# batra-mlp-lab/visdial

Measured on AMD Instinct MI355X. Metric: QA-rounds/sec training mn-att-ques-im-hist+disc (batch 20x10x100), higher is better.
Workload: dtype f32 operands and results; the option recurrence multiplies the EXACT 3-way bf16 split of both operands (9 bf16 MFMA products per fp32 product, f32 accumulate: fp32-grade, errors at the f32 MFMA's own level) -- its two step kernels and its weight-gradient contraction; f32 MFMA (v_mfma_f32_32x32x2_f32

## Files before the change

### visdial_amd/csrc/common.h

```cpp
#pragma once
#include <hip/hip_runtime.h>
#include <stdint.h>
#include <stdio.h>
#include <string.h>

#define VD_OK 0
#define VD_ERR_ARG -1
#define VD_ERR_HIP -2
#define VD_ERR_STATE -3
#define VD_FLAG_BF16 1
#define VD_FLAG_SPLIT9 2
#define VD_FLAG_SPLIT6 4
#define VD_FLAG_SPLIT3 8
#define VD_FLAG_SPLIT (VD_FLAG_SPLIT9 | VD_FLAG_SPLIT6 | VD_FLAG_SPLIT3)
#define VD_FLAG_LIVE_PREFIX 16
#define VD_FLAG_STATE_ONLY 32
#define VD_FLAG_TREE 64
#define VD_LIVE_PREFIX_ROWS 128

void vd_set_error(const char* fmt, ...);

#define VD_CHECK_ARG(cond, ...)                                   \
  do {                                                            \
    if (!(cond)) {                                                \
// ... 41 lines not shown
  int n;
  long quads_per_row;
};
int vd_zero_inactive_multi(const VdZeroSet& z, const int32_t* nact_dev, int T, int N, hipStream_t stream);

typedef unsigned short vd_bf16_bits;
int vd_lstm_forward_c16(const vd_bf16_bits* table16, int64_t tab_ld, const int32_t* tok_gather, const float* Wh, vd_bf16_bits* gates16,
                        vd_bf16_bits* h16, float* h_last, float* c, int T, int N, int H, hipStream_t stream);
int vd_lstm_backward_c16(const float* Wh, vd_bf16_bits* gates16, const float* c, const float* dh_last, float* dc_work, int T, int N, int H,
                         hipStream_t stream);
int vd_f32_to_bf16(const float* src, vd_bf16_bits* dst, int64_t n, hipStream_t stream);
int vd_gemm_tn_acc_bf16(const vd_bf16_bits* A16, const vd_bf16_bits* B16, float* C, int64_t ldc, int M, int N, int K, hipStream_t stream);
int vd_segment_rowsum_acc_bf16(const vd_bf16_bits* X16, int64_t ldx, const int32_t* tok, const int32_t* perm, int64_t n, int ncol,
                               float* out, int64_t ldo, hipStream_t stream);

int vd_bf16_shadow_get(int slot, const float* base, size_t floats, vd_bf16_bits** out);
const vd_bf16_bits* vd_bf16_shadow_find(const float* p, size_t floats);
void vd_bf16_shadow_invalidate(const float* p, size_t floats);

typedef float f32x16 __attribute__((ext_vector_type(16)));

__device__ __forceinline__ float vd_rcp(float x) { return __builtin_amdgcn_rcpf(x); }
__device__ __forceinline__ float vd_sigmoid(float x) { return vd_rcp(1.0f + __expf(-x)); }
__device__ __forceinline__ float vd_tanh(float x) {
  const float e = __expf(-2.0f * fabsf(x));
  const float t = (1.0f - e) * vd_rcp(1.0f + e);
  return copysignf(t, x);
}

typedef unsigned vd_u32x4 __attribute__((ext_vector_type(4)));
// ... 59 lines not shown
```

### visdial_amd/csrc/elementwise.hip

```cpp
#include <stdlib.h>

#include "common.h"

__device__ __forceinline__ uint32_t mix32(uint64_t x) {
  x ^= x >> 33;
  x *= 0xff51afd7ed558ccdULL;
  x ^= x >> 33;
  x *= 0xc4ceb9fe1a85ec53ULL;
  x ^= x >> 33;
  return (uint32_t)x;
}

__global__ void dropout_mask_kernel(uint8_t* __restrict__ mask, long n, uint64_t seed, float p) {
  const long i4 = ((long)blockIdx.x * blockDim.x + threadIdx.x) * 4;
  if (i4 >= n) return;
  const uint32_t thr = (uint32_t)(p * 16777216.0f);
  uint8_t m[4];
#pragma unroll
  for (int k = 0; k < 4; ++k) {
    const uint32_t h = mix32(seed * 0x9E3779B97F4A7C15ULL + (uint64_t)(i4 + k));
    m[k] = ((h >> 8) >= thr) ? 1 : 0;
  }
  if (i4 + 3 < n) {
    *reinterpret_cast<uint32_t*>(mask + i4) = m[0] | (m[1] << 8) | (m[2] << 16) | ((uint32_t)m[3] << 24);
// ... 109 lines not shown
  unsigned long long todo = __ballot(active);
  const int lane = threadIdx.x & 63;
  while (todo) {
    const int leader = __ffsll((long long)todo) - 1;
    const int ltok = __shfl(tok, leader, 64);
    const unsigned long long same = __ballot(active && tok == ltok) & todo;
    int basev = 0;
    if (lane == leader) basev = atomicAdd(base + ltok, __popcll(same));
    basev = __shfl(basev, leader, 64);
    if ((same >> lane) & 1ULL) result = basev + __popcll(same & ((1ULL << lane) - 1ULL));
    todo &= ~same;
  }
  return result;
}

__global__ void tok_count_kernel(const int* __restrict__ tok, long n, int* __restrict__ count) {
  const long i = (long)blockIdx.x * blockDim.x + threadIdx.x;
  const bool active = i < n;
  wave_agg_atomic_inc(count, active ? tok[i] : 0, active);
}

__global__ void tok_scan_kernel(const int* __restrict__ count, int V, int* __restrict__ offset,
                                int* __restrict__ cursor) {
  __shared__ int part[1024];
  const int tid = threadIdx.x, nt = blockDim.x;
  const int per = (V + nt - 1) / nt;
  const int b = tid * per, e = min(V, b + per);
  int s = 0;
  for (int i = b; i < e; ++i) s += count[i];
  part[tid] = s;
  __syncthreads();
  if (tid == 0) {
    int run = 0;
    for (int i = 0; i < nt; ++i) {
      const int t = part[i];
      part[i] = run;
      run += t;
    }
    offset[V] = run;
  }
  __syncthreads();
  int run = part[tid];
  for (int i = b; i < e; ++i) {
    offset[i] = run;
    cursor[i] = run;
    run += count[i];
  }
}

__global__ void tok_fill_kernel(const int* __restrict__ tok, long n, int* __restrict__ cursor,
                                int* __restrict__ perm) {
  const long i = (long)blockIdx.x * blockDim.x + threadIdx.x;
  const bool active = i < n;
  const int p = wave_agg_atomic_inc(cursor, active ? tok[i] : 0, active);
  if (active) perm[p] = (int)i;
}

template <int CHUNK, bool X16 = false>
__global__ void __launch_bounds__(256)
segment_rowsum_kernel(const float* __restrict__ X, long ldx, const int* __restrict__ tok,
                      const int* __restrict__ perm, long n, int ncol, float* __restrict__ out, long ldo) {
  __shared__ int srow[CHUNK], stok[CHUNK];
  const long p0 = (long)blockIdx.x * CHUNK;
  if (p0 >= n) return;
  const int cnt = (int)min((long)CHUNK, n - p0);
  if ((int)threadIdx.x < cnt) {
    const int r = perm[p0 + threadIdx.x];
    srow[threadIdx.x] = r;
    stok[threadIdx.x] = tok[r];
// ... 194 lines not shown
                    float scale, void* stream);
}
int vd_zero_inactive_multi(const VdZeroSet& z, const int32_t* nact_dev, int T, int N, hipStream_t stream) {
  VD_CHECK_ARG(z.n >= 1 && z.n <= 6 && nact_dev && T >= 0 && N >= 0, "vd_zero_inactive_multi: bad args");
  if (T == 0 || N == 0) return VD_OK;
  VdZeroSet zz = z;
  zz.quads_per_row = 0;
  for (int i = 0; i < z.n; ++i) {
    VD_CHECK_ARG(z.buf[i] && z.ncols[i] % 4 == 0, "vd_zero_inactive_multi: buffer %d", i);
    zz.quads_per_row += z.ncols[i] >> 2;
  }
  hipLaunchKernelGGL(zero_inactive_multi_kernel, dim3(128, T), dim3(256), 0, stream, zz, nact_dev, N);
  VD_LAUNCH_CHECK();
  return VD_OK;
}
extern "C" {
int vd_embed_gather(const float* emb, const int32_t* tok, const uint8_t* mask, float* out, int64_t rows, int E,
                    float scale, void* stream) {
  VD_CHECK_ARG(emb && tok && out && rows >= 0 && E > 0 && E % 4 == 0, "vd_embed_gather: bad args (E=%d)", E);
  if (rows == 0) return VD_OK;
  hipLaunchKernelGGL(embed_gather_kernel, grid1d(rows * (E / 4), 256), dim3(256), 0, (hipStream_t)stream, emb,
                     tok, mask, out, (long)rows, E, scale);
  VD_LAUNCH_CHECK();
  return VD_OK;
}

int vd_embed_scatter_acc(float* demb, const int32_t* tok, const uint8_t* mask, const float* dx, int64_t rows,
                         int E, float scale, void* stream) {
  VD_CHECK_ARG(demb && tok && dx && rows >= 0 && E > 0, "vd_embed_scatter_acc: bad args");
  if (rows == 0) return VD_OK;
  hipLaunchKernelGGL(embed_scatter_kernel, grid1d(rows * E, 256), dim3(256), 0, (hipStream_t)stream, demb, tok,
                     mask, dx, (long)rows, E, scale);
  VD_LAUNCH_CHECK();
  return VD_OK;
}

int vd_token_sort(const int32_t* tok, int64_t n, int V, int32_t* offset, int32_t* work, int32_t* perm,
                  void* stream) {
  VD_CHECK_ARG(tok && offset && work && perm && n >= 0 && V > 0, "vd_token_sort: bad args");
  hipStream_t s = (hipStream_t)stream;
  int* count = work;
  int* cursor = work + V;
  VD_HIP(hipMemsetAsync(count, 0, sizeof(int) * V, s));
  if (n > 0) {
    hipLaunchKernelGGL(tok_count_kernel, grid1d(n, 256), dim3(256), 0, s, tok, (long)n, count);
    VD_LAUNCH_CHECK();
  }
  hipLaunchKernelGGL(tok_scan_kernel, dim3(1), dim3(1024), 0, s, count, V, offset, cursor);
  VD_LAUNCH_CHECK();
  if (n > 0) {
    hipLaunchKernelGGL(tok_fill_kernel, grid1d(n, 256), dim3(256), 0, s, tok, (long)n, cursor, perm);
    VD_LAUNCH_CHECK();
  }
  return VD_OK;
}

int vd_segment_rowsum_acc(const float* X, int64_t ldx, const int32_t* tok, const int32_t* perm, int64_t n,
                          int ncol, float* out, int64_t ldo, void* stream) {
  VD_CHECK_ARG(X && tok && perm && out && n >= 0 && ncol > 0 && ncol % 4 == 0 && ldx % 4 == 0 && ldo % 4 == 0,
               "vd_segment_rowsum_acc: bad args");
  if (n == 0) return VD_OK;
  hipLaunchKernelGGL(segment_rowsum_kernel<256>, grid1d(n, 256), dim3(256), 0, (hipStream_t)stream, X, (long)ldx, tok, perm, (long)n, ncol,
                     out, (long)ldo);
  VD_LAUNCH_CHECK();
  return VD_OK;
}

int vd_clamp_adam(float* w, float* g, float* m, float* v, int64_t n, float gscale, float clip, float beta1,
                  float beta2, float eps, float step, void* stream) {
  VD_CHECK_ARG(w && g && m && v && n >= 0, "vd_clamp_adam: bad args");
  VD_CHECK_ARG((((uintptr_t)w | (uintptr_t)g | (uintptr_t)m | (uintptr_t)v) & 15) == 0,
               "vd_clamp_adam: buffers must be 16-byte aligned");
  if (n == 0) return VD_OK;
  hipLaunchKernelGGL(clamp_adam_kernel, grid1d((n + 3) / 4, 256), dim3(256), 0, (hipStream_t)stream, w, g, m, v,
                     (long)n, gscale, clip, beta1, beta2, eps, step);
  VD_LAUNCH_CHECK();
  return VD_OK;
}

}

int vd_segment_rowsum_acc_bf16(const vd_bf16_bits* X16, int64_t ldx, const int32_t* tok, const int32_t* perm, int64_t n, int ncol,
                               float* out, int64_t ldo, hipStream_t stream) {
  VD_CHECK_ARG(X16 && tok && perm && out && n >= 0 && ncol % 4 == 0 && ldx % 4 == 0, "vd_segment_rowsum_acc_bf16: bad args");
  if (n == 0) return VD_OK;
  hipLaunchKernelGGL((segment_rowsum_kernel<256, true>), grid1d(n, 256), dim3(256), 0, stream, reinterpret_cast<const float*>(X16), (long)ldx,
                     tok, perm, (long)n, ncol, out, (long)ldo);
  VD_LAUNCH_CHECK();
  return VD_OK;
}
```

### visdial_amd/csrc/lstm.hip

```cpp
#include "gemm_core.h"
#include "split_core.h"

extern "C" int vd_gemm_tn_acc(const float* A, int64_t lda, const float* B, int64_t ldb, float* C, int64_t ldc, int M,
                              int N, int K, int flags, void* stream);

template <int SEQ, bool C16 = false>
struct EpiLstmFwdT {
  const float* xproj;
  long xld;
  const int* tok_gather;
  const int* tok_mask;
  const float* c_prev;
  float* gates;
  float* c_out;
  float* h_out;
  int H;
  vd_bf16_bits* h16 = nullptr;
  __device__ __forceinline__ void sequential(const f32x16 (&acc)[4], int row0, int vcol0, int lane, int M, float* scr) const {
    const int j = (vcol0 >> 7) * 32 + (lane & 7) * 4;
    float4 ai[4], af[4], ao[4], ag[4];
    tile_to_rows(acc[0], scr, lane, ai);
    tile_to_rows(acc[1], scr, lane, af);
    tile_to_rows(acc[2], scr, lane, ao);
    tile_to_rows(acc[3], scr, lane, ag);
// ... 396 lines not shown
      L.g16[3] = __builtin_amdgcn_raw_buffer_load_b64(R.g, og4 >> 1, 3 * (uH4 >> 1), 0);
    } else {
    L.g[0] = vd_buf_ld4(R.g, og4, 0);
    L.g[1] = vd_buf_ld4(R.g, og4, uH4);
    L.g[2] = vd_buf_ld4(R.g, og4, 2 * uH4);
    L.g[3] = vd_buf_ld4(R.g, og4, 3 * uH4);
    }
    L.ct = vd_buf_ld4(R.ct, o4, 0);
    const float4 z = make_float4(0.f, 0.f, 0.f, 0.f);
    L.cp = c_prev ? vd_buf_ld4(R.cp, o4, 0) : z;
    L.dcv = dc_first ? z : vd_buf_ld4(R.dc, o4, 0);
    L.dhx = (dh_a || dh_b) ? vd_buf_ld4(R.dh1, o4, 0) : z;
  }
  __device__ __forceinline__ void operator()(const f32x16 (&acc)[NT], int row0, int col0, int lane, int M,
                                             int N, float* scr) const {
    const int rl = lane >> 3, cl = (lane & 7) * 4;
    const bool two_dh = TWO && dh_a && dh_b;
    const Rsrc R{vd_rsrc(gates), vd_rsrc(c_t), vd_rsrc(c_prev), vd_rsrc(dc), vd_rsrc(dh_a ? dh_a : dh_b), vd_rsrc(dh_b), vd_rsrc(da16)};
    const unsigned uH4 = (unsigned)H * 4u;
#pragma unroll
    for (int jt = 0; jt < NT; ++jt) {
      float4 d4[4];
      tile_to_rows(acc[jt], scr, lane, d4);
      if (jt == 0) VD_T(3);
      const int j = col0 + jt * 32 + cl;
      const int jc = j < N ? j : N - 4;
#pragma unroll
      for (int pp = 0; pp < 4; pp += BATCH) {
        Slot L[BATCH];
        unsigned o4[BATCH], og4[BATCH];
#pragma unroll
        for (int q = 0; q < BATCH; ++q) {
          const int row = row0 + (pp + q) * 8 + rl;
          o4[q] = (unsigned)(row < M ? row : M - 1) * uH4 + (unsigned)jc * 4u;
          og4[q] = 4u * o4[q] - 12u * (unsigned)jc;
          load_slot_buf(L[q], R, o4[q], og4[q], uH4);
        }
        __builtin_amdgcn_sched_barrier(0);
#pragma unroll
        for (int q = 0; q < BATCH; ++q) {
          Slot& C = L[q];
// ... 38 lines not shown
              vd_buf_st4_bf16(R.g, og4[q] >> 1, 3 * (uH4 >> 1), ag);
            } else {
            vd_buf_st4(R.g, og4[q], 0, ai);
            vd_buf_st4(R.g, og4[q], uH4, af);
            vd_buf_st4(R.g, og4[q], 2 * uH4, ao);
            vd_buf_st4(R.g, og4[q], 3 * uH4, ag);
            }
            vd_buf_st4(R.dc, o4[q], 0, dn);
            if (!C16 && da16) {
              vd_buf_st4_bf16(R.g16, og4[q] >> 1, 0, ai);
              vd_buf_st4_bf16(R.g16, og4[q] >> 1, uH4 >> 1, af);
              vd_buf_st4_bf16(R.g16, og4[q] >> 1, uH4, ao);
              vd_buf_st4_bf16(R.g16, og4[q] >> 1, 3 * (uH4 >> 1), ag);
            }
          }
        }
      }
    }
  }
};

using CfgF9 = GemmCfg<4, 1, 4, 16, 0, 4, 41984>;
using CfgB1 = GemmCfg<4, 1, 4, 32, 0, 3>;
using CfgB11 = GemmCfg<4, 1, 2, 16, 0, 4, 41984>;
using CfgFbf16 = GemmCfg<4, 1, 4, 32, 0, 3, 0, 1>;
using CfgBbf16 = GemmCfg<4, 1, 2, 32, 0, 3, 0, 1>;
#ifndef VD_C16_LDS
#define VD_C16_LDS 41984
#endif
using CfgF9bf16 = GemmCfg<4, 1, 4, 16, 0, 4, VD_C16_LDS, 1>;
using CfgB11bf16 = GemmCfg<4, 1, 2, 16, 0, 4, VD_C16_LDS, 1>;
using CfgFwdSmallA = GemmCfg<1, 4, 4, 8, 0, 3>;
using CfgFwdSmallC = GemmCfg<1, 4, 4, 8, 0, 4>;
using CfgBwdSmallD = GemmCfg<1, 4, 1, 32, 2, 4>;
using CfgTickFwdBf16 = GemmCfg<1, 4, 4, 16, 0, 3, 0, 1>;
using CfgTickBwdBf16 = GemmCfg<1, 4, 1, 32, 0, 4, 0, 1>;

__global__ void __launch_bounds__(256) wh_gate_transpose_kernel(const float* __restrict__ Wh,
                                                                float* __restrict__ WhT, int H, int plain = 0) {
// ... 36 lines not shown
  SrcKGate4 b{Wh, 4L * H, H};
  if (N >= VD_THROUGHPUT_ROWS) return launch_gemm<CfgF9>(N, 4 * H, K, 1, a, b, epi, s);
  return launch_gemm<CfgFwdSmallA>(N, 4 * H, K, 1, a, b, epi, s);
}

static int lstm_step_fwd_tree(const float* h_prev, const float* Wh, int N, int H, const EpiLstmFwdTree& epi, hipStream_t s) {
  SrcRowTree a{h_prev, H, epi.tok_mask, epi.parent};
  SrcKGate4 b{Wh, 4L * H, H};
  if (N >= VD_THROUGHPUT_ROWS) return launch_gemm<CfgF9>(N, 4 * H, H, 1, a, b, epi, s);
  return launch_gemm<CfgFwdSmallA>(N, 4 * H, H, 1, a, b, epi, s);
}

static int lstm_step_bwd(const float* da_next, const float* Wh, int N, int H, int K, const float* dh_a,
                         const float* dh_b, float* gates, const float* c_t, const float* c_prev, float* dc,
                         int dc_first, hipStream_t s, int split = 0, const vd_bf16_bits* W3 = nullptr, vd_bf16_bits* da16 = nullptr,
                         const vd_bf16_bits* da16_next = nullptr, const vd_bf16_bits* Wh16 = nullptr) {
  SrcRow a{da_next, 4L * H};
  SrcRow b{Wh, 4L * H};
  if (split && K > 0 && !(dh_a && dh_b)) {
    EpiLstmBwd<4, 2, false> e{dh_a, dh_b, gates, c_t, c_prev, dc, dc_first, H};
    if (split == 9) return launch_gemm_split<9>(N, H, K, da_next, 4L * H, W3, 4L * H, 4L * H * H, e, s);
    if (split == 6) return launch_gemm_split<6>(N, H, K, da_next, 4L * H, W3, 4L * H, 4L * H * H, e, s);
    return launch_gemm_split<3>(N, H, K, da_next, 4L * H, W3, 4L * H, 4L * H * H, e, s);
  }
  if (da16 && K > 0) {
    EpiLstmBwd<2> e{dh_a, dh_b, gates, c_t, c_prev, dc, dc_first, H, da16};
    if (da16_next && Wh16 && K % 32 == 0)
      return launch_gemm_glds<CfgB11bf16, false>(N, H, K / 2, 1, reinterpret_cast<const float*>(da16_next), 2L * H,
                                                 reinterpret_cast<const float*>(Wh16), 2L * H, e, s);
    return launch_gemm<CfgBbf16>(N, H, K, 1, a, b, e, s);
  }
  if (da16) {
    EpiLstmBwd<2> e{dh_a, dh_b, gates, c_t, c_prev, dc, dc_first, H, da16};
// ... 297 lines not shown
      rc = launch_gemm_split<6>(N, 4 * H, H, hp, (long)H, W3, (long)H, 4L * H * H, e, s);
    else if (split == 3)
      rc = launch_gemm_split<3>(N, 4 * H, H, hp, (long)H, W3, (long)H, 4L * H * H, e, s);
    else if (glds)
      rc = launch_gemm_glds<CfgF9, false>(N, 4 * H, H, 1, hp, (long)H, WhT, (long)H, e, s);
    else
      rc = lstm_step_fwd(hp, Wh, N, H, H, e, s);
    if (rc) return rc;
  }
  return VD_OK;
}

int vd_lstm_backward(const float* Wh, float* gates, const float* c, const float* c0, const float* dh_seq,
                     const float* dh_last, const float* dc_last, float* dc_work, float* dh0, const float* h_seq,
                     float* dWh_acc, int T, int N, int H, int flags, void* stream) {
  VD_CHECK_ARG(T >= 1 && N >= 0 && H > 0 && H % 32 == 0, "vd_lstm_backward: bad dims T=%d N=%d H=%d", T, N, H);
  VD_CHECK_ARG(Wh && gates && c && dc_work, "vd_lstm_backward: null pointer");
  VD_CHECK_ARG((h_seq == nullptr) == (dWh_acc == nullptr), "vd_lstm_backward: h_seq and dWh_acc go together");
  VD_CHECK_ARG((long)N * 4 * H * 4 < (1L << 32), "vd_lstm_backward: N=%d rows x 4H=%d exceed 4 GB per step: split the batch", N, 4 * H);
  hipStream_t s = (hipStream_t)stream;
  const long NH = (long)N * H;
  if (dc_last && dc_last != dc_work) VD_HIP(hipMemcpyAsync(dc_work, dc_last, NH * sizeof(float), hipMemcpyDeviceToDevice, s));
  const bool bf16 = (flags & VD_FLAG_BF16) && vd_lstm_bf16_fits(N, H);
  const int split = !bf16 && T > 1 && vd_lstm_glds_bwd_fits(N, H) ? vd_split_nprod(flags) : 0;
  vd_bf16_bits* da16 = nullptr;
  vd_bf16_bits* Wh16 = nullptr;
  if (bf16) {
    if (int rc0 = vd_bf16_shadow_get(1, gates, (size_t)T * 4 * NH, &da16)) return rc0;
    if (T > 1) {
      VdStreamScratch wscr;
      if (int rc0 = vd_stream_scratch(s, (size_t)4 * H * H * 6, 0, &wscr)) return rc0;
// ... 4 lines not shown
    vd_bf16_shadow_invalidate(gates, (size_t)T * 4 * NH);
  }
  const vd_bf16_bits* W3 = nullptr;
  if (split) {
    VdStreamScratch wscr;
    if (int rc0 = vd_stream_scratch(s, (size_t)4 * H * H * 10, 0, &wscr)) return rc0;
    vd_bf16_bits* w3 = reinterpret_cast<vd_bf16_bits*>(wscr.wht + (size_t)4 * H * H);
    if (int rc0 = weights_to_bf16x3(Wh, w3, 4L * H * H, s)) return rc0;
    W3 = w3;
  }
  for (int t = T - 1; t >= 0; --t) {
    const bool last = (t == T - 1);
    const float* da_next = last ? nullptr : gates + (long)(t + 1) * 4 * NH;
    const int rc = lstm_step_bwd(da_next, Wh, N, H, last ? 0 : 4 * H, dh_seq ? dh_seq + t * NH : nullptr, (last && dh_last) ? dh_last : nullptr,
                                 gates + (long)t * 4 * NH, c + t * NH, t ? c + (t - 1) * NH : c0, dc_work, (last && !dc_last) ? 1 : 0, s, split,
                                 W3, da16 ? da16 + (long)t * 4 * NH : nullptr, (da16 && !last) ? da16 + (long)(t + 1) * 4 * NH : nullptr, Wh16);
    if (rc) return rc;
  }
  int rc = VD_OK;
  if (dWh_acc && T > 1) {
    rc = vd_gemm_tn_acc(h_seq, H, gates + 4 * NH, 4L * H, dWh_acc, 4L * H, H, 4 * H, (T - 1) * N, flags & (VD_FLAG_BF16 | VD_FLAG_SPLIT9), s);
    if (rc) return rc;
  }
  if (dh0) {
    SrcRow a{gates, 4L * H};
    SrcRow b{Wh, 4L * H};
    EpiStore<4> e{dh0, H, nullptr, VD_ACT_NONE, 0};
    rc = launch_gemm<CfgB1>(N, H, 4 * H, 1, a, b, e, s);
    if (rc) return rc;
  }
  return VD_OK;
}

}

template <class Cfg>
static int lstm2_forward_ticks(const vd_lstm2_fwd_t* st, int nstacks, int H, int Tmax, hipStream_t stream) {
  for (int tau = 0; tau < Tmax + 2; ++tau) {
    GroupArgs<TickFwdProb, 3 * VD_MAX_STACKS> g;
    g.nprob = 0;
    for (int s = 0; s < nstacks; ++s) {
      const vd_lstm2_fwd_t& S = st[s];
      const long NH = (long)S.N * H;
      for (int layer = 1; layer <= 2; ++layer) {
        const int t = layer == 1 ? tau : tau - 2;
        if (t < 0 || t >= S.T) continue;
        float* gates = layer == 1 ? S.gates1 : S.gates2;
        float* h = layer == 1 ? S.h1 : S.h2;
        float* c = layer == 1 ? S.c1 : S.c2;
// ... 133 lines not shown
```

### visdial_amd/csrc/paths.h

```cpp
#pragma once
#include "common.h"

static inline int vd_precision_flags(int lstmBf16) {
  switch (lstmBf16) {
    case 0: return 0;
    case 1: return VD_FLAG_BF16;
    case 3: return VD_FLAG_SPLIT3;
    case 6: return VD_FLAG_SPLIT6;
    case 9: return VD_FLAG_SPLIT9;
    default: return -1;
  }
}
static inline int vd_split_nprod(int flags) {
  return (flags & VD_FLAG_SPLIT9) ? 9 : (flags & VD_FLAG_SPLIT6) ? 6 : (flags & VD_FLAG_SPLIT3) ? 3 : 0;
}

constexpr long VD_THROUGHPUT_ROWS = 2048;
constexpr int VD_LSTM_FWD_TILE_BIG = 128, VD_LSTM_FWD_TILE_SMALL = 32;
static inline int vd_lstm_fwd_row_tile(long N) { return N >= VD_THROUGHPUT_ROWS ? VD_LSTM_FWD_TILE_BIG : VD_LSTM_FWD_TILE_SMALL; }
static inline bool vd_lstm_glds_fwd_fits(long N, int H) { return N >= VD_THROUGHPUT_ROWS && H % 32 == 0 && N * H * 4 < (1L << 32); }
static inline bool vd_lstm_glds_bwd_fits(long N, int H) { return N >= VD_THROUGHPUT_ROWS && H % 32 == 0 && N * 4 * H * 4 < (1L << 32); }
static inline bool vd_lstm_bf16_fits(long N, int H) { return N >= VD_THROUGHPUT_ROWS && H % 32 == 0; }
static inline bool vd_lstm_c16_fits(long N, int H) { return N >= VD_THROUGHPUT_ROWS && H % 128 == 0; }

static inline bool vd_tn_kmajor_fits(long M, long N, long K) { return M % 128 == 0 && N % 128 == 0 && K >= 1024; }
constexpr int VD_SPLIT_TN_BM = 256, VD_SPLIT_TN_BN = 128;
static inline bool vd_tn_split_tiles(long M, long N) { return M % VD_SPLIT_TN_BM == 0 && N % VD_SPLIT_TN_BN == 0; }

static inline bool vd_img_split_ok(long rows, int H, int Kc) {
  return rows >= 128 && H % 16 == 0 && Kc % 16 == 0 && rows * (H > Kc ? H : Kc) * 4 < (1L << 32);
}

static inline bool vd_lhood_fused_fits(long rows, long ldh, long V, long ldw, int H) {
  return H >= 64 && H % 16 == 0 && V >= 128 && ldh % 4 == 0 && ldw % 4 == 0 && rows * ldh * 4 < (1L << 32) && V * ldw * 4 < (1L << 32);
}
static inline bool vd_lhood_prefix_fits(int T, long rows) { return T >= 1 && T < 256 && rows >= 1; }
// ... 1 lines not shown
```

### visdial_amd/csrc/rt_core.h

```cpp
#pragma once
#include <math.h>
#include <stdarg.h>
#include <stdlib.h>
#include <string.h>

#include <algorithm>
#include <map>
#include <memory>
#include <numeric>
#include <random>
#include <string>
#include <vector>

#include "../../include/visdial_hip.h"
#include "common.h"
#include "paths.h"

int vd_lstm2_forward_p(const vd_lstm2_fwd_t* st, int nstacks, int H, int flags, hipStream_t stream);
int vd_lstm2_backward_p(const vd_lstm2_bwd_t* st, int nstacks, int H, int flags, hipStream_t stream);

int vd_img_drop_gather(const float* pre, const uint8_t* mask1, float* xdrop, int N, int R, int S2, int H, float scale, hipStream_t stream);
int vd_img_common_forward_p(const float* pre, const uint8_t* mask1, const float* xdrop, const float* Wc, const float* bc, const float* qc,
                            const uint8_t* mask2, float* iqc, int N, int R, int S2, int H, int Kc, float scale, int flags, hipStream_t stream);
int vd_img_tr_backward_p(const float* dz, const float* Wc, const float* p, const float* datt, const uint8_t* mask1, float* dpre, int N, int R,
// ... 53 lines not shown
  int32_t *enode = nullptr, *etgt = nullptr;
};

struct BatchSlot {
  int B = 0;
  bool tree_ok = false;
  std::vector<TreeChunk> tree;
  SeqTok q, h, opt, ain, aout, oin, oout;
  float* img = nullptr;
  int32_t* gt = nullptr;
  std::vector<int32_t> gt_host;
  bool has_gt = false;
  int32_t* opt_uid = nullptr;
  int opt_total = 0;
  int32_t *opt_sort_off = nullptr, *opt_sort_perm = nullptr;
  bool cached = false;
  uint64_t cache_stamp = 0;
  std::vector<int32_t> miss_keys, opt_host;
  hipEvent_t ready = nullptr;
  hipEvent_t done = nullptr;
  bool used = false;
  bool uploaded = false;
  std::map<std::string, DevBuf> bufs, pinned;
};

struct RowIndex {
  int T = 0;
  std::vector<int32_t> keys;
  std::vector<int32_t> table;
  int32_t size() const { return T ? (int32_t)(keys.size() / (size_t)T) : 0; }
// ... 476 lines not shown
```

### visdial_amd/csrc/rt_decoders.h

```cpp
#pragma once
#include "rt_encoders.h"

namespace vdrt {

int option_cache_resolve(vd_model* m, BatchSlot& sl, const int32_t* options, long NO, int To, hipStream_t s);

struct Decoder {
  virtual ~Decoder() {}
  virtual void declare(vd_model* m) = 0;
  virtual int forward_backward(vd_model* m, BatchSlot& b, bool only_forward) = 0;
  virtual int retrieve(vd_model* m, BatchSlot& b) = 0;
  virtual int retrieve_lhood(vd_model*, BatchSlot&) {
    vd_set_error("vd_model_retrieve_lhood: the live-row log-likelihood head scores candidates of decoder 'gen'; this model's decoder is 'disc'");
    return VD_ERR_ARG;
  }
  virtual int gen_begin(vd_model*, const int32_t*, int) { return no_gen(); }
  virtual int gen_step(vd_model*, const int32_t*, float*) { return no_gen(); }
  virtual int gen_select(vd_model*, const int32_t*, int) { return no_gen(); }
  virtual int gen_beam_search(vd_model*, int, int, int, int, int32_t*, double*) { return no_gen(); }
  virtual int gen_sample(vd_model*, int, int, int, double, const double*, int32_t*, double*) { return no_gen(); }
  static int no_gen() {
    vd_set_error("sampling / beam search only for the generative decoder (model.lua:436-438)");
    return VD_ERR_STATE;
  }
// ... 88 lines not shown
    VD_TRY(vd_score_ce(optH, enc_out, b.gt, scores, loss_rows, dedup ? d_optH_full : d_optH, d_enc, N, O, (int)H, 1.0f / N, s));
    if (dedup && !only_forward) {
      VD_TRY(vd_memset(d_optH, 0, (long)NO * H * 4, s));
      VD_TRY(vd_embed_scatter_acc(d_optH, b.opt_uid, nullptr, d_optH_full, NOfull, (int)H, 1.f, s));
    }
    VD_TRY(stage_loss(m, loss_rows, N, false, s));
    m->scores = scores;
    m->prof_valid = !only_forward;
    if (only_forward) return VD_OK;
    VD_TRY(fork_stream(m, s, se));
    float *dc, *dtab;
    int32_t* perm = b.opt_sort_perm;
    VD_TRY(ws_get(m, "opt.dc", (size_t)NO * H, &dc));
    VD_TRY(ws_get(m, "opt.dtable", (size_t)(V + 1) * 4 * H, &dtab));
    VD_CHECK_ARG(perm, "decoder 'disc': the batch slot carries no option-token sort");
    VD_TRY(fork_stream(m, s, st));
    VD_TRY(vd_memset(dtab, 0, (V + 1) * 4 * H * 4, st));
    VD_HIP(hipEventRecord(m->ev_prof[2], s));
    m->wg_active = m->streams && m->s_wg && (flags & VD_FLAG_BF16) != 0;
    m->wg_used = false;
    auto enc_bwd = [&]() -> int {
      VdRange r("encoder backward");
      VD_TRY(m->enc->backward(m, se, b, d_enc));
      VD_PROBE_REC(1, se);
      if (m->wg_used) VD_PROBE_REC(2, m->s_wg);
      if (m->wg_used) {
        VD_TRY(fork_stream(m, se, m->s_wg));
        VD_HIP(hipEventRecord(m->ev_enc_grads, m->s_wg));
      } else {
        VD_HIP(hipEventRecord(m->ev_enc_grads, se));
      }
      m->enc_grads_recorded = true;
      return VD_OK;
    };
    {
      VdRange r("disc: option LSTM backward");
      if (c16) VD_TRY(vd_lstm_backward_c16(Wopt + E * 4 * H, gates16, c, d_optH, dc, To, NO, (int)H, s));
      else VD_TRY(vd_lstm_backward(Wopt + E * 4 * H, gates, c, nullptr, nullptr, d_optH, nullptr, dc, nullptr, nullptr, nullptr, To, NO, (int)H, flags, s));
    }
    VD_HIP(hipEventRecord(m->ev_prof[3], s));
    VD_TRY(enc_bwd());
    VdRange rwg("disc: table gradient + dWh");
    VD_TRY(fork_stream(m, s, st));
    if (c16) VD_TRY(vd_segment_rowsum_acc_bf16(gates16, 4 * H, b.opt.tok, perm, (long)To * NO, (int)(4 * H), dtab, 4 * H, st));
    else VD_TRY(vd_segment_rowsum_acc(gates, 4 * H, b.opt.tok, perm, (long)To * NO, (int)(4 * H), dtab, 4 * H, st));
    VD_TRY(vd_colsum_acc(dtab, 4 * H, (int)V + 1, (int)(4 * H), Gp(m, "opt.b"), st));
    VD_TRY(vd_gemm_tn_acc(Wp(m, "embed"), E, dtab, 4 * H, Gp(m, "opt.W"), 4 * H, (int)E, (int)(4 * H), (int)V + 1, 0, st));
    VD_HIP(hipEventRecord(m->ev_prof[4], s));
    if (To > 1 && c16)
      VD_TRY(vd_gemm_tn_acc_bf16(h16, gates16 + (long)NO * 4 * H, Gp(m, "opt.W") + E * 4 * H, 4 * H, (int)H, (int)(4 * H), (To - 1) * NO, s));
    else if (To > 1)
      VD_TRY(vd_gemm_tn_acc(h, H, gates + (long)NO * 4 * H, 4 * H, Gp(m, "opt.W") + E * 4 * H, 4 * H, (int)H, (int)(4 * H), (To - 1) * NO,
                            flags & (VD_FLAG_BF16 | VD_FLAG_SPLIT9), s));
    VD_HIP(hipEventRecord(m->ev_prof[5], s));
    VD_TRY(vd_gemm_nt(dtab, 4 * H, Wopt, 4 * H, nullptr, Gp(m, "embed"), E, (int)V + 1, (int)E, (int)(4 * H), VD_ACT_NONE, 2, st));
    VD_PROBE_REC(3, st);
    VD_TRY(join_stream(m, se, s));
    if (m->wg_used) VD_TRY(join_stream(m, m->s_wg, s));
    m->wg_active = m->wg_used = false;
    VD_TRY(join_stream(m, st, s));
// ... 540 lines not shown
```

### visdial_amd/csrc/runtime.hip

```cpp
#include "rt_decoders.h"

using namespace vdrt;

vd_model::~vd_model() {}

namespace {

int upload_tokens(BatchSlot& sl, SeqTok& ss, const std::string& tag, const int32_t* rows_major, int N, int T, bool sorted, hipStream_t s) {
  ss.T = T;
  ss.N = N;
  ss.present = true;
  ss.sorted = sorted;
  const size_t TN = (size_t)T * N;
  const size_t total = sorted ? 7 * TN + 2 * (size_t)N + T : TN;
  int32_t* stage = nullptr;
  VD_TRY(pin_get(sl.pinned, tag + ".stage", total * sizeof(int32_t), (void**)&stage));
  int32_t* tok = stage;
  std::vector<int> len(sorted ? N : 0);
  for (int n = 0; n < N; ++n) {
    int first = T;
    for (int t = 0; t < T; ++t) {
      const int32_t v = rows_major[(size_t)n * T + t];
      tok[(size_t)t * N + n] = v;
      if (v != 0 && first == T) first = t;
// ... 488 lines not shown
  if (m->use_hist) VD_TRY(upload_tokens(sl, sl.h, "h", hb->hist, N, hb->Th, m->is_graph || hist_wave, s));
  if (m->use_im) {
    const size_t img_n = (size_t)hb->B * (m->is_att ? (size_t)m->p.imgSpatialSize * m->p.imgSpatialSize : 1) * m->p.imgFeatureSize;
    float* ip = nullptr;
    VD_TRY(pin_get(sl.pinned, "img.stage", img_n * sizeof(float), (void**)&ip));
    memcpy(ip, hb->img_feat, img_n * sizeof(float));
    VD_TRY(dev_get(sl.bufs, "img", img_n * sizeof(float), (void**)&sl.img));
    VD_HIP(hipMemcpyAsync(sl.img, ip, img_n * sizeof(float), hipMemcpyHostToDevice, s));
  }
  if (disc) {
    sl.opt_uid = nullptr;
    sl.opt_total = (int)NO;
    sl.cached = false;
    const int To = hb->To;
    bool dedup = false;
    if (m->ocache.capacity > 0 && !m->training) {
      sl.opt_host.assign(hb->options, hb->options + (size_t)NO * To);
      VD_TRY(option_cache_resolve(m, sl, sl.opt_host.data(), NO, To, s));
    } else if (NO > 1) {
      std::vector<int32_t> uid((size_t)NO), uniq;
      uniq.reserve((size_t)NO * To);
      const size_t cap = (size_t)1 << (64 - __builtin_clzll((unsigned long long)(2 * NO)));
      std::vector<int32_t> table(cap, -1);
      int U = 0;
      for (long r = 0; r < NO; ++r) {
        const int32_t* row = hb->options + (size_t)r * To;
        uint64_t h = 1469598103934665603ull;
        for (int t = 0; t < To; ++t) h = (h ^ (uint32_t)row[t]) * 1099511628211ull;
        size_t pos = (size_t)(h ^ (h >> 29)) & (cap - 1);
        for (;;) {
          const int32_t u = table[pos];
          if (u < 0) {
            table[pos] = U;
            uid[r] = U++;
            uniq.insert(uniq.end(), row, row + To);
            break;
          }
          if (memcmp(uniq.data() + (size_t)u * To, row, (size_t)To * sizeof(int32_t)) == 0) {
            uid[r] = u;
            break;
          }
          pos = (pos + 1) & (cap - 1);
        }
      }
      if ((double)U <= 0.95 * (double)NO) {
        dedup = true;
        VD_TRY(upload_tokens(sl, sl.opt, "opt", uniq.data(), U, To, false, s));
        int32_t* up = nullptr;
        VD_TRY(pin_get(sl.pinned, "opt.uid.stage", (size_t)NO * sizeof(int32_t), (void**)&up));
        memcpy(up, uid.data(), (size_t)NO * sizeof(int32_t));
        VD_TRY(dev_get(sl.bufs, "opt.uid", (size_t)NO * sizeof(int32_t), (void**)&sl.opt_uid));
        VD_HIP(hipMemcpyAsync(sl.opt_uid, up, (size_t)NO * sizeof(int32_t), hipMemcpyHostToDevice, s));
      }
    }
    if (!dedup && !sl.cached) VD_TRY(upload_tokens(sl, sl.opt, "opt", hb->options, (int)NO, hb->To, false, s));
    sl.opt_sort_off = sl.opt_sort_perm = nullptr;
    if (!sl.cached) {
      const long V1 = (long)m->p.vocabSize + 1, n = (long)sl.opt.T * sl.opt.N;
      int32_t* work;
      VD_TRY(dev_get(sl.bufs, "opt.sort_off", (size_t)(V1 + 1) * sizeof(int32_t), (void**)&sl.opt_sort_off));
      VD_TRY(dev_get(sl.bufs, "opt.sort_work", (size_t)2 * V1 * sizeof(int32_t), (void**)&work));
      VD_TRY(dev_get(sl.bufs, "opt.sort_perm", (size_t)n * sizeof(int32_t), (void**)&sl.opt_sort_perm));
      VD_TRY(vd_token_sort(sl.opt.tok, n, (int)V1, sl.opt_sort_off, work, sl.opt_sort_perm, s));
    }
  }
  if (!disc && hb->answer_in && hb->answer_out) {
    VD_TRY(upload_tokens(sl, sl.ain, "ain", hb->answer_in, N, hb->Ta, false, s));
    VD_TRY(upload_tokens(sl, sl.aout, "aout", hb->answer_out, N, hb->Ta, false, s));
  }
  sl.tree_ok = false;
  if (!disc && hb->option_in && hb->option_out) {
    VD_TRY(upload_tokens(sl, sl.oin, "oin", hb->option_in, (int)NO, hb->To, false, s));
    VD_TRY(upload_tokens(sl, sl.oout, "oout", hb->option_out, (int)NO, hb->To, false, s));
    if (m->lhood_tree) VD_TRY(build_lhood_tree(m, sl, hb->option_in, hb->option_out, N, O, hb->To, s));
  }
  sl.has_gt = hb->answer_ind != nullptr;
  sl.gt_host.assign(N, 0);
  int32_t* gp = nullptr;
// ... 195 lines not shown
```

Measured before the change: 8134.

## Fold pad-token table gradient into option LSTM backward step epilogue

The option-LSTM backward step epilogue now sums the gate gradients of pad-token rows (token 0) and accumulates them directly into the embedding-table gradient row 0, first in LDS and then with global atomics. The token sort skips pad tokens, so the later segment row-sum touches only non-pad cells. This removes the pad rows, often the majority of option tokens, from the separate gather-and-sum pass. In exchange it adds atomic traffic, a block barrier and LDS work to every backward step, and it needs a host-side pad count.

```diff
diff --git a/visdial_amd/csrc/common.h b/visdial_amd/csrc/common.h
--- a/visdial_amd/csrc/common.h
+++ b/visdial_amd/csrc/common.h
@@ -79,6 +79,11 @@
 int vd_segment_rowsum_acc_bf16(const vd_bf16_bits* X16, int64_t ldx, const int32_t* tok, const int32_t* perm, int64_t n, int ncol,
                                float* out, int64_t ldo, hipStream_t stream);
 
+int vd_lstm_backward_padsum(const float* Wh, float* gates, const float* c, const float* c0, const float* dh_seq, const float* dh_last,
+                            const float* dc_last, float* dc_work, float* dh0, const float* h_seq, float* dWh_acc, int T, int N, int H, int flags,
+                            const int32_t* pad_tok, float* pad_dst, hipStream_t stream);
+int vd_token_sort_nopad(const int32_t* tok, int64_t n, int V, int32_t* offset, int32_t* work, int32_t* perm, hipStream_t stream);
+
 int vd_bf16_shadow_get(int slot, const float* base, size_t floats, vd_bf16_bits** out);
 const vd_bf16_bits* vd_bf16_shadow_find(const float* p, size_t floats);
 void vd_bf16_shadow_invalidate(const float* p, size_t floats);
diff --git a/visdial_amd/csrc/elementwise.hip b/visdial_amd/csrc/elementwise.hip
--- a/visdial_amd/csrc/elementwise.hip
+++ b/visdial_amd/csrc/elementwise.hip
@@ -147,10 +147,12 @@
   return result;
 }
 
+template <bool NOPAD = false>
 __global__ void tok_count_kernel(const int* __restrict__ tok, long n, int* __restrict__ count) {
   const long i = (long)blockIdx.x * blockDim.x + threadIdx.x;
-  const bool active = i < n;
-  wave_agg_atomic_inc(count, active ? tok[i] : 0, active);
+  const int t = i < n ? tok[i] : 0;
+  const bool active = i < n && (!NOPAD || t != 0);
+  wave_agg_atomic_inc(count, t, active);
 }
 
 __global__ void tok_scan_kernel(const int* __restrict__ count, int V, int* __restrict__ offset,
@@ -181,11 +183,13 @@
   }
 }
 
+template <bool NOPAD = false>
 __global__ void tok_fill_kernel(const int* __restrict__ tok, long n, int* __restrict__ cursor,
                                 int* __restrict__ perm) {
   const long i = (long)blockIdx.x * blockDim.x + threadIdx.x;
-  const bool active = i < n;
-  const int p = wave_agg_atomic_inc(cursor, active ? tok[i] : 0, active);
+  const int t = i < n ? tok[i] : 0;
+  const bool active = i < n && (!NOPAD || t != 0);
+  const int p = wave_agg_atomic_inc(cursor, t, active);
   if (active) perm[p] = (int)i;
 }
 
@@ -410,6 +414,25 @@
   VD_LAUNCH_CHECK();
   return VD_OK;
 }
+template <bool NOPAD>
+static int token_sort(const int32_t* tok, int64_t n, int V, int32_t* offset, int32_t* work, int32_t* perm, hipStream_t s) {
+  VD_CHECK_ARG(tok && offset && work && perm && n >= 0 && V > 0, "vd_token_sort: bad args");
+  int* count = work;
+  int* cursor = work + V;
+  VD_HIP(hipMemsetAsync(count, 0, sizeof(int) * V, s));
+  if (n > 0) {
+    hipLaunchKernelGGL(tok_count_kernel<NOPAD>, grid1d(n, 256), dim3(256), 0, s, tok, (long)n, count);
+    VD_LAUNCH_CHECK();
+  }
+  hipLaunchKernelGGL(tok_scan_kernel, dim3(1), dim3(1024), 0, s, count, V, offset, cursor);
+  VD_LAUNCH_CHECK();
+  if (n > 0) {
+    hipLaunchKernelGGL(tok_fill_kernel<NOPAD>, grid1d(n, 256), dim3(256), 0, s, tok, (long)n, cursor, perm);
+    VD_LAUNCH_CHECK();
+  }
+  return VD_OK;
+}
+
 extern "C" {
 int vd_embed_gather(const float* emb, const int32_t* tok, const uint8_t* mask, float* out, int64_t rows, int E,
                     float scale, void* stream) {
@@ -433,22 +456,7 @@
 
 int vd_token_sort(const int32_t* tok, int64_t n, int V, int32_t* offset, int32_t* work, int32_t* perm,
                   void* stream) {
-  VD_CHECK_ARG(tok && offset && work && perm && n >= 0 && V > 0, "vd_token_sort: bad args");
-  hipStream_t s = (hipStream_t)stream;
-  int* count = work;
-  int* cursor = work + V;
-  VD_HIP(hipMemsetAsync(count, 0, sizeof(int) * V, s));
-  if (n > 0) {
-    hipLaunchKernelGGL(tok_count_kernel, grid1d(n, 256), dim3(256), 0, s, tok, (long)n, count);
-    VD_LAUNCH_CHECK();
-  }
-  hipLaunchKernelGGL(tok_scan_kernel, dim3(1), dim3(1024), 0, s, count, V, offset, cursor);
-  VD_LAUNCH_CHECK();
-  if (n > 0) {
-    hipLaunchKernelGGL(tok_fill_kernel, grid1d(n, 256), dim3(256), 0, s, tok, (long)n, cursor, perm);
-    VD_LAUNCH_CHECK();
-  }
-  return VD_OK;
+  return token_sort<false>(tok, n, V, offset, work, perm, (hipStream_t)stream);
 }
 
 int vd_segment_rowsum_acc(const float* X, int64_t ldx, const int32_t* tok, const int32_t* perm, int64_t n,
@@ -476,6 +484,10 @@
 
 }
 
+int vd_token_sort_nopad(const int32_t* tok, int64_t n, int V, int32_t* offset, int32_t* work, int32_t* perm, hipStream_t stream) {
+  return token_sort<true>(tok, n, V, offset, work, perm, stream);
+}
+
 int vd_segment_rowsum_acc_bf16(const vd_bf16_bits* X16, int64_t ldx, const int32_t* tok, const int32_t* perm, int64_t n, int ncol,
                                float* out, int64_t ldo, hipStream_t stream) {
   VD_CHECK_ARG(X16 && tok && perm && out && n >= 0 && ncol % 4 == 0 && ldx % 4 == 0, "vd_segment_rowsum_acc_bf16: bad args");
diff --git a/visdial_amd/csrc/lstm.hip b/visdial_amd/csrc/lstm.hip
--- a/visdial_amd/csrc/lstm.hip
+++ b/visdial_amd/csrc/lstm.hip
@@ -434,7 +434,21 @@
   }
   __device__ __forceinline__ void operator()(const f32x16 (&acc)[NT], int row0, int col0, int lane, int M,
                                              int N, float* scr) const {
+    run<false>(acc, row0, col0, lane, M, N, scr, nullptr, 0, 0);
+  }
+  template <bool PAD>
+  __device__ __forceinline__ void run(const f32x16 (&acc)[NT], int row0, int col0, int lane, int M, int N, float* scr, float* pad_dst,
+                                      int pad0, int pad1) const {
     const int rl = lane >> 3, cl = (lane & 7) * 4;
+    unsigned padw = 0;
+    bool tile_pad = false;
+    int wv = 0;
+    if constexpr (PAD) {
+      wv = __builtin_amdgcn_readfirstlane((int)threadIdx.x >> 6);
+      const unsigned long long b0 = __ballot(pad0 != 0), b1 = __ballot(pad1 != 0);
+      tile_pad = (b0 | b1) != 0ull;
+      padw = (unsigned)(((wv & 2) ? b1 : b0) >> ((wv & 1) * 32));
+    }
     const bool two_dh = TWO && dh_a && dh_b;
     const Rsrc R{vd_rsrc(gates), vd_rsrc(c_t), vd_rsrc(c_prev), vd_rsrc(dc), vd_rsrc(dh_a ? dh_a : dh_b), vd_rsrc(dh_b), vd_rsrc(da16)};
     const unsigned uH4 = (unsigned)H * 4u;
@@ -445,6 +459,13 @@
       if (jt == 0) VD_T(3);
       const int j = col0 + jt * 32 + cl;
       const int jc = j < N ? j : N - 4;
+      if constexpr (PAD) {
+        if (padw != 0) {
+#pragma unroll
+          for (int g = 0; g < 4; ++g) *reinterpret_cast<float4*>(scr + (rl * 4 + g) * 32 + cl) = make_float4(0.f, 0.f, 0.f, 0.f);
+          asm volatile("" ::: "memory");
+        }
+      }
 #pragma unroll
       for (int pp = 0; pp < 4; pp += BATCH) {
         Slot L[BATCH];
@@ -513,15 +534,87 @@
               vd_buf_st4_bf16(R.g16, og4[q] >> 1, 3 * (uH4 >> 1), ag);
             }
           }
+          if constexpr (PAD) {
+            if (((padw >> ((pp + q) * 8 + rl)) & 1u) != 0 && j < N) {
+              float* cell = scr + rl * 128 + cl;
+#define VD_PADADD(g, v)                                                                                   \
+              unsafeAtomicAdd(cell + g * 32, v.x); unsafeAtomicAdd(cell + g * 32 + 1, v.y);                 \
+              unsafeAtomicAdd(cell + g * 32 + 2, v.z); unsafeAtomicAdd(cell + g * 32 + 3, v.w);
+              VD_PADADD(0, ai) VD_PADADD(1, af) VD_PADADD(2, ao) VD_PADADD(3, ag)
+#undef VD_PADADD
+            }
+          }
         }
       }
-    }
+      if constexpr (PAD) {
+        if (tile_pad) {
+          float2 t = make_float2(0.f, 0.f);
+          if (padw != 0) {
+            asm volatile("" ::: "memory");
+#pragma unroll
+            for (int r = 0; r < 8; ++r) {
+              const float2 u = *reinterpret_cast<const float2*>(scr + r * 128 + lane * 2);
+              t.x += u.x;
+              t.y += u.y;
+            }
+            asm volatile("" ::: "memory");
+          }
+          *reinterpret_cast<float2*>(scr + (4 - wv) * 1024 + wv * 512 + jt * 128 + lane * 2) = t;
+        }
+      }
+    }
+    if constexpr (PAD) {
+      if (tile_pad) {
+        __syncthreads();
+        const int c2 = (int)threadIdx.x * 2;
+        if (c2 < NT * 128) {
+          const float* all = scr + (4 - wv) * 1024 + c2;
+          float2 t = *reinterpret_cast<const float2*>(all);
+#pragma unroll
+          for (int w = 1; w < 4; ++w) {
+            const float2 u = *reinterpret_cast<const float2*>(all + w * 512);
+            t.x += u.x;
+            t.y += u.y;
+          }
+          const int jt = c2 >> 7, g = (c2 >> 5) & 3, u = col0 + jt * 32 + (c2 & 31);
+          if (u < N) {
+            unsafeAtomicAdd(pad_dst + g * H + u, t.x);
+            unsafeAtomicAdd(pad_dst + g * H + u + 1, t.y);
+          }
+        }
+      }
+    }
+  }
+};
+constexpr int PAD_LDS_FLOATS = 4 * 1024 + 4 * 512;
+
+template <int NT, int BATCH = (NT == 1 ? 2 : 1), bool TWO = true>
+struct EpiLstmBwdPad : EpiLstmBwd<NT, BATCH, TWO, false> {
+  const int* tok;
+  float* pad_dst;
+  static_assert(NT == 2 || NT == 4, "throughput tiles only");
+  struct Pre {
+    int t0, t1;
+  };
+  __device__ __forceinline__ void preload(Pre& q, int row0, int lane, int M) const {
+    const int r0 = row0 - (__builtin_amdgcn_readfirstlane((int)threadIdx.x >> 6)) * 32 + lane, r1 = r0 + 64;
+    q.t0 = r0 < M ? tok[r0] : 1;
+    q.t1 = r1 < M ? tok[r1] : 1;
+  }
+  __device__ __forceinline__ void operator()(const f32x16 (&acc)[NT], int row0, int col0, int lane, int M, int N, float* scr,
+                                             const Pre* pre = nullptr) const {
+    Pre q;
+    if (pre) q = *pre;
+    else preload(q, row0, lane, M);
+    this->template run<true>(acc, row0, col0, lane, M, N, scr, pad_dst, q.t0 == 0, q.t1 == 0);
   }
 };
 
 using CfgF9 = GemmCfg<4, 1, 4, 16, 0, 4, 41984>;
 using CfgB1 = GemmCfg<4, 1, 4, 32, 0, 3>;
 using CfgB11 = GemmCfg<4, 1, 2, 16, 0, 4, 41984>;
+static_assert(CfgB11::LDS_BYTES >= PAD_LDS_FLOATS * 4 && SplitCfg::LDS_BYTES >= PAD_LDS_FLOATS * 4 && CfgB11::BM == 128 && CfgB11::WM == 4 &&
+                  SplitCfg::BM == 128 && SplitCfg::WM == 4, "EpiLstmBwdPad: 128-row four-wave tiles, LDS behind the four scratch areas");
 using CfgFbf16 = GemmCfg<4, 1, 4, 32, 0, 3, 0, 1>;
 using CfgBbf16 = GemmCfg<4, 1, 2, 32, 0, 3, 0, 1>;
 #ifndef VD_C16_LDS
@@ -588,9 +681,25 @@
 static int lstm_step_bwd(const float* da_next, const float* Wh, int N, int H, int K, const float* dh_a,
                          const float* dh_b, float* gates, const float* c_t, const float* c_prev, float* dc,
                          int dc_first, hipStream_t s, int split = 0, const vd_bf16_bits* W3 = nullptr, vd_bf16_bits* da16 = nullptr,
-                         const vd_bf16_bits* da16_next = nullptr, const vd_bf16_bits* Wh16 = nullptr) {
+                         const vd_bf16_bits* da16_next = nullptr, const vd_bf16_bits* Wh16 = nullptr, const int* pad_tok = nullptr,
+                         float* pad_dst = nullptr) {
   SrcRow a{da_next, 4L * H};
   SrcRow b{Wh, 4L * H};
+  if (pad_dst) {
+    if (split && K > 0 && !(dh_a && dh_b)) {
+      EpiLstmBwdPad<4, 2, false> e{{dh_a, dh_b, gates, c_t, c_prev, dc, dc_first, H}, pad_tok, pad_dst};
+      if (split == 9) return launch_gemm_split<9>(N, H, K, da_next, 4L * H, W3, 4L * H, 4L * H * H, e, s);
+      if (split == 6) return launch_gemm_split<6>(N, H, K, da_next, 4L * H, W3, 4L * H, 4L * H * H, e, s);
+      return launch_gemm_split<3>(N, H, K, da_next, 4L * H, W3, 4L * H, 4L * H * H, e, s);
+    }
+    if (K > 0 && !(dh_a && dh_b)) {
+      EpiLstmBwdPad<2, 2, false> e2c{{dh_a, dh_b, gates, c_t, c_prev, dc, dc_first, H}, pad_tok, pad_dst};
+      return launch_gemm_glds<CfgB11, false>(N, H, K, 1, da_next, 4L * H, Wh, 4L * H, e2c, s);
+    }
+    EpiLstmBwdPad<2> e{{dh_a, dh_b, gates, c_t, c_prev, dc, dc_first, H}, pad_tok, pad_dst};
+    if (K > 0) return launch_gemm_glds<CfgB11, false>(N, H, K, 1, da_next, 4L * H, Wh, 4L * H, e, s);
+    return launch_gemm<CfgB11>(N, H, K, 1, a, b, e, s);
+  }
   if (split && K > 0 && !(dh_a && dh_b)) {
     EpiLstmBwd<4, 2, false> e{dh_a, dh_b, gates, c_t, c_prev, dc, dc_first, H};
     if (split == 9) return launch_gemm_split<9>(N, H, K, da_next, 4L * H, W3, 4L * H, 4L * H * H, e, s);
@@ -918,7 +1027,20 @@
 int vd_lstm_backward(const float* Wh, float* gates, const float* c, const float* c0, const float* dh_seq,
                      const float* dh_last, const float* dc_last, float* dc_work, float* dh0, const float* h_seq,
                      float* dWh_acc, int T, int N, int H, int flags, void* stream) {
+  return vd_lstm_backward_padsum(Wh, gates, c, c0, dh_seq, dh_last, dc_last, dc_work, dh0, h_seq, dWh_acc, T, N, H, flags, nullptr, nullptr,
+                                 (hipStream_t)stream);
+}
+
+}
+
+int vd_lstm_backward_padsum(const float* Wh, float* gates, const float* c, const float* c0, const float* dh_seq,
+                            const float* dh_last, const float* dc_last, float* dc_work, float* dh0, const float* h_seq,
+                            float* dWh_acc, int T, int N, int H, int flags, const int32_t* pad_tok, float* pad_dst, hipStream_t stream) {
   VD_CHECK_ARG(T >= 1 && N >= 0 && H > 0 && H % 32 == 0, "vd_lstm_backward: bad dims T=%d N=%d H=%d", T, N, H);
+  VD_CHECK_ARG((pad_tok == nullptr) == (pad_dst == nullptr), "vd_lstm_backward_padsum: pad_tok and pad_dst go together");
+  VD_CHECK_ARG(!pad_dst || vd_lstm_padsum_fits(N, H, flags),
+               "vd_lstm_backward_padsum: the step epilogue sums the pad rows in the fp32 / exact-split throughput kernels only (rows >= %ld, "
+               "no VD_FLAG_BF16); N=%d H=%d flags=%d", VD_THROUGHPUT_ROWS, N, H, flags);
   VD_CHECK_ARG(Wh && gates && c && dc_work, "vd_lstm_backward: null pointer");
   VD_CHECK_ARG((h_seq == nullptr) == (dWh_acc == nullptr), "vd_lstm_backward: h_seq and dWh_acc go together");
   VD_CHECK_ARG((long)N * 4 * H * 4 < (1L << 32), "vd_lstm_backward: N=%d rows x 4H=%d exceed 4 GB per step: split the batch", N, 4 * H);
@@ -953,7 +1075,8 @@
     const float* da_next = last ? nullptr : gates + (long)(t + 1) * 4 * NH;
     const int rc = lstm_step_bwd(da_next, Wh, N, H, last ? 0 : 4 * H, dh_seq ? dh_seq + t * NH : nullptr, (last && dh_last) ? dh_last : nullptr,
                                  gates + (long)t * 4 * NH, c + t * NH, t ? c + (t - 1) * NH : c0, dc_work, (last && !dc_last) ? 1 : 0, s, split,
-                                 W3, da16 ? da16 + (long)t * 4 * NH : nullptr, (da16 && !last) ? da16 + (long)(t + 1) * 4 * NH : nullptr, Wh16);
+                                 W3, da16 ? da16 + (long)t * 4 * NH : nullptr, (da16 && !last) ? da16 + (long)(t + 1) * 4 * NH : nullptr, Wh16,
+                                 pad_tok ? pad_tok + (long)t * N : nullptr, pad_dst);
     if (rc) return rc;
   }
   int rc = VD_OK;
@@ -971,7 +1094,7 @@
   return VD_OK;
 }
 
-}
+
 
 template <class Cfg>
 static int lstm2_forward_ticks(const vd_lstm2_fwd_t* st, int nstacks, int H, int Tmax, hipStream_t stream) {
diff --git a/visdial_amd/csrc/paths.h b/visdial_amd/csrc/paths.h
--- a/visdial_amd/csrc/paths.h
+++ b/visdial_amd/csrc/paths.h
@@ -20,6 +20,7 @@
 static inline int vd_lstm_fwd_row_tile(long N) { return N >= VD_THROUGHPUT_ROWS ? VD_LSTM_FWD_TILE_BIG : VD_LSTM_FWD_TILE_SMALL; }
 static inline bool vd_lstm_glds_fwd_fits(long N, int H) { return N >= VD_THROUGHPUT_ROWS && H % 32 == 0 && N * H * 4 < (1L << 32); }
 static inline bool vd_lstm_glds_bwd_fits(long N, int H) { return N >= VD_THROUGHPUT_ROWS && H % 32 == 0 && N * 4 * H * 4 < (1L << 32); }
+static inline bool vd_lstm_padsum_fits(long N, int H, int flags) { return !(flags & VD_FLAG_BF16) && vd_lstm_glds_bwd_fits(N, H); }
 static inline bool vd_lstm_bf16_fits(long N, int H) { return N >= VD_THROUGHPUT_ROWS && H % 32 == 0; }
 static inline bool vd_lstm_c16_fits(long N, int H) { return N >= VD_THROUGHPUT_ROWS && H % 128 == 0; }
 
diff --git a/visdial_amd/csrc/rt_core.h b/visdial_amd/csrc/rt_core.h
--- a/visdial_amd/csrc/rt_core.h
+++ b/visdial_amd/csrc/rt_core.h
@@ -91,6 +91,7 @@
   int32_t* opt_uid = nullptr;
   int opt_total = 0;
   int32_t *opt_sort_off = nullptr, *opt_sort_perm = nullptr;
+  long opt_npad = -1;
   bool cached = false;
   uint64_t cache_stamp = 0;
   std::vector<int32_t> miss_keys, opt_host;
diff --git a/visdial_amd/csrc/rt_decoders.h b/visdial_amd/csrc/rt_decoders.h
--- a/visdial_amd/csrc/rt_decoders.h
+++ b/visdial_amd/csrc/rt_decoders.h
@@ -126,8 +126,16 @@
     VD_TRY(ws_get(m, "opt.dc", (size_t)NO * H, &dc));
     VD_TRY(ws_get(m, "opt.dtable", (size_t)(V + 1) * 4 * H, &dtab));
     VD_CHECK_ARG(perm, "decoder 'disc': the batch slot carries no option-token sort");
+    const long npad = c16 ? -1 : b.opt_npad;
+    VD_CHECK_ARG(npad < 0 || (vd_lstm_padsum_fits(NO, (int)H, flags) && npad <= (long)To * NO),
+                 "decoder 'disc': the batch slot's option-token sort does not match the step (%ld pad cells)", npad);
     VD_TRY(fork_stream(m, s, st));
-    VD_TRY(vd_memset(dtab, 0, (V + 1) * 4 * H * 4, st));
+    if (npad >= 0) {
+      VD_TRY(vd_memset(dtab, 0, 4 * H * 4, s));
+      VD_TRY(vd_memset(dtab + 4 * H, 0, V * 4 * H * 4, st));
+    } else {
+      VD_TRY(vd_memset(dtab, 0, (V + 1) * 4 * H * 4, st));
+    }
     VD_HIP(hipEventRecord(m->ev_prof[2], s));
     m->wg_active = m->streams && m->s_wg && (flags & VD_FLAG_BF16) != 0;
     m->wg_used = false;
@@ -148,14 +156,15 @@
     {
       VdRange r("disc: option LSTM backward");
       if (c16) VD_TRY(vd_lstm_backward_c16(Wopt + E * 4 * H, gates16, c, d_optH, dc, To, NO, (int)H, s));
-      else VD_TRY(vd_lstm_backward(Wopt + E * 4 * H, gates, c, nullptr, nullptr, d_optH, nullptr, dc, nullptr, nullptr, nullptr, To, NO, (int)H, flags, s));
+      else VD_TRY(vd_lstm_backward_padsum(Wopt + E * 4 * H, gates, c, nullptr, nullptr, d_optH, nullptr, dc, nullptr, nullptr, nullptr, To, NO, (int)H,
+                                          flags, npad >= 0 ? b.opt.tok : nullptr, npad >= 0 ? dtab : nullptr, s));
     }
     VD_HIP(hipEventRecord(m->ev_prof[3], s));
     VD_TRY(enc_bwd());
     VdRange rwg("disc: table gradient + dWh");
     VD_TRY(fork_stream(m, s, st));
     if (c16) VD_TRY(vd_segment_rowsum_acc_bf16(gates16, 4 * H, b.opt.tok, perm, (long)To * NO, (int)(4 * H), dtab, 4 * H, st));
-    else VD_TRY(vd_segment_rowsum_acc(gates, 4 * H, b.opt.tok, perm, (long)To * NO, (int)(4 * H), dtab, 4 * H, st));
+    else VD_TRY(vd_segment_rowsum_acc(gates, 4 * H, b.opt.tok, perm, (long)To * NO - std::max(npad, 0L), (int)(4 * H), dtab, 4 * H, st));
     VD_TRY(vd_colsum_acc(dtab, 4 * H, (int)V + 1, (int)(4 * H), Gp(m, "opt.b"), st));
     VD_TRY(vd_gemm_tn_acc(Wp(m, "embed"), E, dtab, 4 * H, Gp(m, "opt.W"), 4 * H, (int)E, (int)(4 * H), (int)V + 1, 0, st));
     VD_HIP(hipEventRecord(m->ev_prof[4], s));
diff --git a/visdial_amd/csrc/runtime.hip b/visdial_amd/csrc/runtime.hip
--- a/visdial_amd/csrc/runtime.hip
+++ b/visdial_amd/csrc/runtime.hip
@@ -526,6 +526,7 @@
     sl.cached = false;
     const int To = hb->To;
     bool dedup = false;
+    long npad_all = 0, npad_uniq = 0;
     if (m->ocache.capacity > 0 && !m->training) {
       sl.opt_host.assign(hb->options, hb->options + (size_t)NO * To);
       VD_TRY(option_cache_resolve(m, sl, sl.opt_host.data(), NO, To, s));
@@ -538,7 +539,12 @@
       for (long r = 0; r < NO; ++r) {
         const int32_t* row = hb->options + (size_t)r * To;
         uint64_t h = 1469598103934665603ull;
-        for (int t = 0; t < To; ++t) h = (h ^ (uint32_t)row[t]) * 1099511628211ull;
+        int zeros = 0;
+        for (int t = 0; t < To; ++t) {
+          h = (h ^ (uint32_t)row[t]) * 1099511628211ull;
+          zeros += row[t] == 0;
+        }
+        npad_all += zeros;
         size_t pos = (size_t)(h ^ (h >> 29)) & (cap - 1);
         for (;;) {
           const int32_t u = table[pos];
@@ -546,6 +552,7 @@
             table[pos] = U;
             uid[r] = U++;
             uniq.insert(uniq.end(), row, row + To);
+            npad_uniq += zeros;
             break;
           }
           if (memcmp(uniq.data() + (size_t)u * To, row, (size_t)To * sizeof(int32_t)) == 0) {
@@ -567,13 +574,21 @@
     }
     if (!dedup && !sl.cached) VD_TRY(upload_tokens(sl, sl.opt, "opt", hb->options, (int)NO, hb->To, false, s));
     sl.opt_sort_off = sl.opt_sort_perm = nullptr;
+    sl.opt_npad = -1;
     if (!sl.cached) {
       const long V1 = (long)m->p.vocabSize + 1, n = (long)sl.opt.T * sl.opt.N;
       int32_t* work;
       VD_TRY(dev_get(sl.bufs, "opt.sort_off", (size_t)(V1 + 1) * sizeof(int32_t), (void**)&sl.opt_sort_off));
       VD_TRY(dev_get(sl.bufs, "opt.sort_work", (size_t)2 * V1 * sizeof(int32_t), (void**)&work));
       VD_TRY(dev_get(sl.bufs, "opt.sort_perm", (size_t)n * sizeof(int32_t), (void**)&sl.opt_sort_perm));
-      VD_TRY(vd_token_sort(sl.opt.tok, n, (int)V1, sl.opt_sort_off, work, sl.opt_sort_perm, s));
+      if (vd_lstm_padsum_fits(sl.opt.N, m->p.rnnHiddenSize, m->flags)) {
+        if (NO <= 1)
+          for (long i = 0; i < NO * To; ++i) npad_all += hb->options[i] == 0;
+        sl.opt_npad = dedup ? npad_uniq : npad_all;
+        VD_TRY(vd_token_sort_nopad(sl.opt.tok, n, (int)V1, sl.opt_sort_off, work, sl.opt_sort_perm, s));
+      } else {
+        VD_TRY(vd_token_sort(sl.opt.tok, n, (int)V1, sl.opt_sort_off, work, sl.opt_sort_perm, s));
+      }
     }
   }
   if (!disc && hb->answer_in && hb->answer_out) {
```

Result: slower. 7804 (-4.1%).
